# torognes/vsearch

Hardware: NVIDIA H100
Metric: usearch_global_gcups (higher is better)
Workload: dtype int16

## Files before the change

vsearch_b200/csrc/align_ckpt.cuh:

```cuda
#pragma once

#include "align_kernels.cuh"

namespace vsg {

#ifndef VSG_CK_CHUNK
#define VSG_CK_CHUNK 32
#endif
constexpr int CK_CHUNK = VSG_CK_CHUNK;
static_assert(CK_CHUNK == 16 || CK_CHUNK == 32, "chunk");

__host__ __device__ inline size_t ck_row_index(int s, int l) { return (static_cast<size_t>(s >> 2) * 32 + l) * 4 + (s & 3); }
__host__ __device__ inline size_t ck_row_elems(int dmax) { return static_cast<size_t>((dmax + 31 + 3) >> 2) * 128; }
__host__ __device__ inline size_t ck_col_index(int k, int l, int r, int R) { return (static_cast<size_t>(k - 1) * R + r) * 32 + l; }
__host__ __device__ inline size_t ck_col_elems(int dmax, int R) { return static_cast<size_t>((dmax + 31 + CK_CHUNK - 1) / CK_CHUNK) * R * 32; }

enum { CK_PROF = 0, CK_LUT = 1, CK_GEN = 2 };
__host__ __device__ constexpr size_t ck_dyn_smem(int R, int mode)
{
  return mode == CK_PROF ? static_cast<size_t>(FAST_WARPS) * 16 * ((R + 3) / 4) * 32 * 16 : 0;
}

template <int R, int MODE>
__global__ void __launch_bounds__(FAST_WARPS * 32)
nw_ckpt_kernel(const __grid_constant__ ScoreParams sp, DevSeqs qs, DevSeqs ts,
               const FastTask * __restrict__ tasks, int ntasks,
               uint2 * __restrict__ rowck, uint2 * __restrict__ colck, int32_t * __restrict__ stats)
{
  constexpr bool PROF = (MODE == CK_PROF);
  constexpr bool GENERAL = (MODE == CK_GEN);
  static_assert(!PROF || R <= 8, "the per-lane profile is for R <= 8");
  constexpr int RQ = (R + 3) / 4;
  constexpr int LUT_WORDS = GENERAL ? 4096 : (PROF ? 32 : 64 * 32);
  extern __shared__ uint4 prof_mem[];
  __shared__ uint32_t lut[LUT_WORDS];
  __shared__ uint32_t ringX[FAST_WARPS][2 * RING];
  __shared__ uint2 ringA[FAST_WARPS][2 * RING];

  int const lane = threadIdx.x & 31;
  int const wib = threadIdx.x >> 5;

  if (!PROF) {
    for (int e = threadIdx.x; e < LUT_WORDS; e += blockDim.x) {
      if (GENERAL) {
        int const q = e >> 8, dlo = e & 15, dhi = (e >> 4) & 15;
        lut[e] = pk2(-sp.S[dlo][q], -sp.S[dhi][q]);
      } else {
        int const ent = e >> 5;
        int const q = 1 << (ent >> 4), dlo = 1 << (ent & 3), dhi = 1 << ((ent >> 2) & 3);
        lut[e] = pk2(-sp.S[dlo][q], -sp.S[dhi][q]);
      }
    }
    __syncthreads();
  }

  int const w = blockIdx.x * FAST_WARPS + wib;
  if (w >= ntasks) { return; }
  FastTask const tk = tasks[w];

  int const Q = qs.len[tk.q];
  uint8_t const * __restrict__ qsym = qs.sym + qs.off[tk.q];
  int const Dlo = ts.len[tk.tlo], Dhi = ts.len[tk.thi];
  uint8_t const * __restrict__ dlo_p = ts.sym + ts.off[tk.tlo];
  uint8_t const * __restrict__ dhi_p = ts.sym + ts.off[tk.thi];
  int const dmax = tk.dmax;
  int const nsteps = dmax + 31;

  int const QRqi = sp.go[Q_I] + sp.ge[Q_I], Rqi = sp.ge[Q_I];
  int const QRqr = sp.go[Q_R] + sp.ge[Q_R], Rqr = sp.ge[Q_R];
  int const QRti = sp.go[T_I] + sp.ge[T_I], Rti = sp.ge[T_I];
  int const QRtr = sp.go[T_R] + sp.ge[T_R], Rtr = sp.ge[T_R];
  int const gotl = sp.go[T_L], getl = sp.ge[T_L];
  int const goql = sp.go[Q_L], geql = sp.ge[Q_L];
// ... 117 lines not shown
      __syncwarp();
      if (lane < CK_CHUNK && cc + CK_CHUNK < dmax) { fetch(cc + CK_CHUNK); }
    }
    uint32_t const slot0 = static_cast<uint32_t>(s0 - lane) & (RING - 1);
    constexpr unsigned CH = CK_CHUNK;
    bool const steady = (s0 >= 32) && (s0 + CK_CHUNK - 1 < dmax) &&
                        (static_cast<unsigned>(cap_lo - s0) >= CH) && (static_cast<unsigned>(cap_hi - s0) >= CH) &&
                        (static_cast<unsigned>(Dlo - 1 - (s0 - 31)) >= 31u + CH) && (static_cast<unsigned>(Dhi - 1 - (s0 - 31)) >= 31u + CH);
    if (steady) {
      bool const lo_done = (s0 - 31 > Dlo - 1), hi_done = (s0 - 31 > Dhi - 1);
      uint32_t const yneg = pk2(-(lo_done ? QRtr : QRti), -(hi_done ? QRtr : QRti));
      uint32_t const z = pk2(lo_done ? Rtr : Rti, hi_done ? Rtr : Rti);
      uint32_t const ypos = pk2(lo_done ? QRtr : QRti, hi_done ? QRtr : QRti);
      uint32_t htop = BIAS2 - pk1(goql + (s0 - lane + 1) * geql);
      uint32_t aX = rX_s + slot0 * 4u;
#pragma unroll 1
      for (int k0 = 0; k0 < CK_CHUNK; k0 += 4) {
        uint32_t ho[4], fo[4];
#pragma unroll
        for (int u = 0; u < 4; u++) {
          uint32_t hin = __shfl_up_sync(0xffffffffu, Hout, 1);
          uint32_t fin = __shfl_up_sync(0xffffffffu, Fout, 1);
          uint32_t const x = lds32(aX + (k0 + u) * 4u);
          if (lane == 0) { hin = htop; fin = htop - ypos; }
          htop -= geql2;
          column(x, yneg, z, hin, fin);
          ho[u] = Hout; fo[u] = Fout;
        }
        uint4 * const tp = reinterpret_cast<uint4 *>(myrow + ck_row_index(s0 + k0, lane));
        tp[0] = make_uint4(ho[0], fo[0], ho[1], fo[1]);
        tp[1] = make_uint4(ho[2], fo[2], ho[3], fo[3]);
      }
    } else {
      int const kend = min(CK_CHUNK, nsteps - s0);
      int c = s0 - lane;
      uint32_t aX = rX_s + slot0 * 4u, aA = rA_s + slot0 * 8u;
      for (int k = 0; k < kend; k++, c++, aX += 4u, aA += 8u) {
        uint32_t hin = __shfl_up_sync(0xffffffffu, Hout, 1);
        uint32_t fin = __shfl_up_sync(0xffffffffu, Fout, 1);
        if (c >= 0 && c < dmax) {
          uint32_t const x = lds32(aX);
          uint2 yz;
          asm volatile("ld.shared.v2.u32 {%0,%1}, [%2];" : "=r"(yz.x), "=r"(yz.y) : "r"(aA));
          if (lane == 0) {
            hin = BIAS2 - pk1(goql + (c + 1) * geql);
            fin = __vadd2(hin, yz.x);
          }
          column(x, yz.x, yz.y, hin, fin);
          myrow[ck_row_index(s0 + k, lane)] = make_uint2(Hout, Fout);
          if (capture && (c == Dlo - 1 || c == Dhi - 1)) {
            uint32_t v = 0;
#pragma unroll
            for (int r = 0; r < R; r++) { if (r == rlast) { v = Hl[r]; } }
            if (c == Dlo - 1) { score_lo = static_cast<int>(v & 0xffffu) - static_cast<int>(BIAS); }
            if (c == Dhi - 1) { score_hi = static_cast<int>(v >> 16) - static_cast<int>(BIAS); }
          }
        }
      }
    }
    if (s0 + CK_CHUNK < nsteps) {
      uint2 * const cp = mycol + ck_col_index(s0 / CK_CHUNK + 1, lane, 0, R);
#pragma unroll
      for (int r = 0; r < R; r++) { cp[static_cast<size_t>(r) * 32] = make_uint2(Hl[r], E[r]); }
    }
  }
  if (lane == llast) {
    if (tk.out_lo >= 0) { stats[static_cast<size_t>(tk.out_lo) * VSG_STAT_WORDS + VSG_STAT_SCORE] = score_lo + sp.shift * (Q + Dlo); }
    if (tk.out_hi >= 0) { stats[static_cast<size_t>(tk.out_hi) * VSG_STAT_WORDS + VSG_STAT_SCORE] = score_hi + sp.shift * (Q + Dhi); }
  }
}

}

#include "tb_ckpt.h"

namespace vsg {

static_assert(ckpt::CHUNK == CK_CHUNK && ckpt::RMAX == FAST_RMAX, "tb_ckpt.h and align_ckpt.cuh disagree");

constexpr int TB_CK_THREADS = 128;

// ... 63 lines not shown
  CigarWriter cw;
  cw.text = TEXT;
  cw.end = TEXT ? (cigar_region + pv.Q + pv.D + 1) : nullptr;
  if (TEXT) { *--cw.end = 0; }
  cw.op = 0; cw.run = 0; cw.len = 0;
  ckpt::TbOut o;
  auto emit = [&](char nop, int n) { if (TEXT) { cw.push_n(nop, n); } };
  if (general) { ckpt::traceback<RT, true>(sp, pv, bits, rows, o, emit); }
  else { ckpt::traceback<RT, false>(sp, pv, bits, rows, o, emit); }
  if (TEXT) { cw.flush(); }
  st[VSG_STAT_ALIGNED] = o.aligned; st[VSG_STAT_MATCHES] = o.matches; st[VSG_STAT_MISMATCHES] = o.mismatches;
  st[VSG_STAT_GAPS] = o.gaps; st[VSG_STAT_TRIM_LEFT] = o.trim_left; st[VSG_STAT_TRIM_RIGHT] = o.trim_right;
  st[VSG_STAT_CIGARLEN] = TEXT ? cw.len : 0;
}

constexpr int32_t TB_VERDICT_ACCEPTED = 0x5ca1ab1e;
struct TbGate {
  const int * ids;
  int nids;
  const int32_t * leader_of;
  int phase;
  int iddef;
  double threshold;
};

__device__ __forceinline__ bool tb_leader_accepted(const ckpt::TbOut & o, int Q, int D, int iddef, double threshold)
{
  int const nal = o.aligned, ma = o.matches, mi = o.mismatches, ga = o.gaps;
  int const tql = o.trim_left > 0 ? o.trim_left : 0, ttl = o.trim_left < 0 ? -o.trim_left : 0;
  int tqr = o.trim_right > 0 ? o.trim_right : 0, ttr = o.trim_right < 0 ? -o.trim_right : 0;
  if (tql >= nal) { tqr = 0; }
// ... 101 lines not shown
```

vsearch_b200/csrc/search.cu:

```cuda
#include "vsg_internal.h"
#include "hit_logic.h"

#include <algorithm>
#include <atomic>
#include <cmath>
#include <climits>
#include <cstdint>
#include <cstdlib>
#include <cstring>
#include <thread>
#include <chrono>
#include <cstdio>

namespace vsg {
int rank_enqueue(vsg_ctx * c, const vsg_index * ix, const vsg_seqset * queries, int64_t q0, int64_t nq,
                 int minwordmatches, int tophits, int mask_lower, uint32_t ** d_seqno, uint32_t ** d_count,
                 int32_t ** d_n, int32_t ** d_status);
int seqset_revcomp(vsg_ctx * c, const vsg_seqset * src, int64_t q0, int64_t nq, vsg_seqset ** out);
void rank_collect_time(vsg_ctx * c);
const vsg_seqset * index_db(const vsg_index * ix);
int index_wordlength(const vsg_index * ix);
}

using namespace vsg;
// ... 90 lines not shown
  if (opts->wordlength != index_wordlength(ix)) { Error::set("vsg_search_batch: wordlength differs from the index"); return VSG_EINVAL; }
  if (opts->iddef < 0 || opts->iddef > 4) { Error::set("vsg_search_batch: iddef must be 0..4"); return VSG_EINVAL; }

  int64_t const seqcount = db->d.n;
  int64_t maxaccepts = opts->maxaccepts, maxrejects = opts->maxrejects < 0 ? 32 : opts->maxrejects;
  if (maxaccepts < 0) { Error::set("vsg_search_batch: maxaccepts must not be negative"); return VSG_EINVAL; }
  if (maxaccepts > seqcount || maxaccepts == 0) { maxaccepts = seqcount; }
  if (maxrejects > seqcount || maxrejects == 0) { maxrejects = seqcount; }
  int64_t tophits64 = maxaccepts + maxrejects + MAXDELAYED;
  if (tophits64 > seqcount) { tophits64 = seqcount; }
  int const minwordmatches = opts->minwordmatches < 0 ? minwordmatches_defaults[opts->wordlength] : opts->minwordmatches;
  double const opt_id = opts->id;
  double const opt_weak_id = (opts->id >= 0.0 && opts->weak_id > opts->id) ? opts->id : opts->weak_id;
  int64_t total_pairs = 0, total_cells = 0, aligned_pairs = 0, aligned_cells = 0;
  bool const lazy = opts->lazy != 0;
  bool const tb_force = [] { const char * e = std::getenv("VSG_TB_GATE_FORCE"); return e != nullptr && e[0] == '1'; }();
  bool tb_gate = false;
  {
    vsg_search_opts d;
    vsg_search_opts_default(&d);
    const char * const e = std::getenv("VSG_TB_GATE");
    tb_gate = (e == nullptr || e[0] != '0') && !lazy && !c->sp.fallback &&
              opts->maxsubs == d.maxsubs && opts->maxgaps == d.maxgaps && opts->mincols == d.mincols && opts->maxdiffs == d.maxdiffs &&
              opts->leftjust == 0 && opts->rightjust == 0 && opts->query_cov == d.query_cov && opts->target_cov == d.target_cov &&
              opts->maxid == d.maxid && opts->mid == d.mid && opts->iddef >= 0 && opts->iddef <= 4 && opt_weak_id <= opt_id &&
              opts->unoise == 0;
  }
  for (int64_t q = 0; q < nq; q++) { counts[q] = 0; }
  if (seqcount == 0 || nq == 0) { if (work) { work[0] = work[1] = work[2] = work[3] = 0; } return VSG_OK; }
  if (tophits64 > 1024) { Error::set("vsg_search_batch: maxaccepts+maxrejects+8 > 1024 is not supported on the device ranker"); return VSG_EINVAL; }
  int const tophits = static_cast<int>(tophits64);
// ... 243 lines not shown
          split = 0;
          while (split < n && static_cast<int64_t>(state_of[split]) < bn) { split++; }
        }
        for (int part = 0; part < 2; part++) {
          size_t const lo = part == 0 ? 0 : split, hi = part == 0 ? split : n;
          if (hi <= lo) { continue; }
          const vsg_seqset * qset = part == 0 ? queries : rc_set;
          const int32_t * lead_part = nullptr;
          if (lead != nullptr) {
            lead_tmp.assign(lead + lo, lead + hi);
            if (lo > 0) { for (auto & v : lead_tmp) { if (v >= 0) { v -= static_cast<int32_t>(lo); } } }
            lead_part = lead_tmp.data();
          }
          int const r = align_pairs_gated(c, qset, db, static_cast<int64_t>(hi - lo), Q + lo, T + lo,
                                          o_sc + lo, o_al + lo, o_ma + lo, o_mi + lo, o_ga + lo, o_tr + 4 * lo, nullptr, 0, nullptr,
                                          lead_part, tb_force ? -1.0 : 100.0 * opt_id + 1e-7, opts->iddef);
          if (r != VSG_OK) { return r; }
        }
        return VSG_OK;
      };
      bool const from_cache = tail_mode;
      auto count_extras = [&]() -> size_t {
        size_t extras = 0;
        for (size_t k = 0; k < np; k++) {
          if (k + 1 == np || pstate[k + 1] != pstate[k]) {
            QState const & S = st[static_cast<size_t>(pstate[k])];
            extras += static_cast<size_t>(std::max(0, S.ncand - (lazy ? S.gend : S.hit_count)));
          }
        }
        return extras;
      };
// ... 386 lines not shown
```

vsearch_b200/csrc/vsg_api.cu:

```cuda
#include "align_kernels.cuh"
#include "align_ckpt.cuh"

#include <cub/cub.cuh>

#include <algorithm>
#include <atomic>
#include <cstdio>
#include <cstdlib>
#include <cstring>
#include <map>
#include <mutex>
#include <chrono>

namespace vsg {

static thread_local std::string g_last_error;
void Error::set(const std::string & m) { g_last_error = m; }

static std::atomic<int64_t> g_launches{0};
void count_launch(int n) { g_launches.fetch_add(n, std::memory_order_relaxed); }

namespace {
struct PoolKey { int device; size_t cls; bool operator<(const PoolKey & o) const { return device != o.device ? device < o.device : cls < o.cls; } };
std::mutex g_pool_mutex;
// ... 215 lines not shown
    return VSG_ECUDA;
  }
  *out = guard.release();
  return VSG_OK;
}

extern "C" void vsg_ctx_destroy(vsg_ctx * c)
{
  if (c == nullptr) { return; }
  for (vsg_ctx * ch : c->children) { vsg_ctx_destroy(ch); }
  c->children.clear();
  cudaSetDevice(c->device);
  if (c->stream != nullptr) { cudaStreamSynchronize(c->stream); }
  for (DevBuf * b : {&c->dir, &c->bnd, &c->he, &c->cigar_scratch, &c->cigar_dense, &c->stats,
                     &c->tasks_fast, &c->tasks_exact, &c->pairs, &c->cigar_len, &c->cigar_offs,
                     &c->cub_tmp, &c->rank_tmp, &c->rank_scratch, &c->pre_flags, &c->ticket}) { b->release(); }
  for (PinBuf * b : {&c->h_tasks, &c->h_stats}) { b->release(); }
  for (auto & ev : c->ev) { if (ev != nullptr) { cudaEventDestroy(ev); } }
  for (auto & ev : c->ev_pool) { cudaEventDestroy(ev); }
  if (c->stream != nullptr) { cudaStreamDestroy(c->stream); }
  delete c;
}

extern "C" int vsg_ctx_set_fallback(vsg_ctx * c, vsg_fallback_fn fn, void * user)
{
  if (c == nullptr) { return VSG_EINVAL; }
  c->fallback = fn;
  c->fallback_user = user;
  return VSG_OK;
}

// ... 161 lines not shown
    return;
  }
  switch (R) {
#define VSG_CASE(r) case r: launch_fast_one<r, false, false>(c, qs, ts, d_tasks, n); break;
    VSG_CASE(1) VSG_CASE(2) VSG_CASE(3) VSG_CASE(4) VSG_CASE(5) VSG_CASE(6) VSG_CASE(7) VSG_CASE(8)
#undef VSG_CASE
#define VSG_CASE(r) case r: if (multi) { launch_fast_one<r, false, true>(c, qs, ts, d_tasks, n); } \
                            else { launch_fast_one<r, false, false>(c, qs, ts, d_tasks, n); } break;
    VSG_CASE(9) VSG_CASE(10) VSG_CASE(11) VSG_CASE(12) VSG_CASE(13) VSG_CASE(14) VSG_CASE(15)
    default: if (multi) { launch_fast_one<16, false, true>(c, qs, ts, d_tasks, n); }
             else { launch_fast_one<16, false, false>(c, qs, ts, d_tasks, n); } break;
#undef VSG_CASE
  }
}

template <int R, int MODE>
void launch_ckpt_one(vsg_ctx * c, const DevSeqs & qs, const DevSeqs & ts, const FastTask * d_tasks, int n)
{
  int const blocks = (n + FAST_WARPS - 1) / FAST_WARPS;
  constexpr size_t dyn = ck_dyn_smem(R, MODE);
  if (dyn > 48 * 1024) {
    cudaFuncSetAttribute(nw_ckpt_kernel<R, MODE>, cudaFuncAttributeMaxDynamicSharedMemorySize, static_cast<int>(dyn));
  }
  nw_ckpt_kernel<R, MODE><<<blocks, FAST_WARPS * 32, dyn, c->stream>>>(
      c->sp2, qs, ts, d_tasks, n, static_cast<uint2 *>(c->dir.p), static_cast<uint2 *>(c->bnd.p),
      static_cast<int32_t *>(c->stats.p));
  count_launch();
}

void launch_ckpt(vsg_ctx * c, int R, bool general, const DevSeqs & qs, const DevSeqs & ts, const FastTask * d_tasks, int n)
{
  if (general) {
    switch (R) {
      case 4: launch_ckpt_one<4, CK_GEN>(c, qs, ts, d_tasks, n); break;
      case 8: launch_ckpt_one<8, CK_GEN>(c, qs, ts, d_tasks, n); break;
      default: launch_ckpt_one<16, CK_GEN>(c, qs, ts, d_tasks, n); break;
    }
    return;
  }
  static const bool force_lut = std::getenv("VSG_CK_LUT") != nullptr;
  if (force_lut && R == 8) { launch_ckpt_one<8, CK_LUT>(c, qs, ts, d_tasks, n); return; }
  switch (R) {
#define VSG_CASE(r) case r: launch_ckpt_one<r, CK_PROF>(c, qs, ts, d_tasks, n); break;
    VSG_CASE(1) VSG_CASE(2) VSG_CASE(3) VSG_CASE(4) VSG_CASE(5) VSG_CASE(6) VSG_CASE(7) VSG_CASE(8)
#undef VSG_CASE
#define VSG_CASE(r) case r: launch_ckpt_one<r, CK_LUT>(c, qs, ts, d_tasks, n); break;
    VSG_CASE(9) VSG_CASE(10) VSG_CASE(11) VSG_CASE(12) VSG_CASE(13) VSG_CASE(14) VSG_CASE(15)
    default: launch_ckpt_one<16, CK_LUT>(c, qs, ts, d_tasks, n); break;
#undef VSG_CASE
  }
}

int launch_tb_ckpt_tasks(vsg_ctx * c, int R, bool general, const DevSeqs & qs, const DevSeqs & ts, const FastTask * d_tasks, int n,
                         const TbGate & gate)
{
  int rc;
  if ((rc = c->ticket.reserve(64)) != VSG_OK) { return rc; }
  VSG_CUDA_OK(cudaMemsetAsync(c->ticket.p, 0, sizeof(int), c->stream));
  int sms = 132;
  cudaDeviceGetAttribute(&sms, cudaDevAttrMultiProcessorCount, c->device);
  int const nthr = gate.ids != nullptr ? gate.nids : 2 * n;
  if (nthr == 0) { return VSG_OK; }
  int const want = (nthr + TB_CK_THREADS - 1) / TB_CK_THREADS;
// ... 8 lines not shown
        c->sp2, qs, ts, d_tasks, n, R, general ? 1 : 0, static_cast<const uint2 *>(c->dir.p), static_cast<const uint2 *>(c->bnd.p),
        static_cast<int32_t *>(c->stats.p), static_cast<int *>(c->ticket.p), tbase, gate);
  } else {
    cudaFuncSetAttribute(traceback_ckpt_tasks_kernel<16>, cudaFuncAttributeMaxDynamicSharedMemorySize, static_cast<int>(tb_ck_smem(16)));
    int per_sm = 1;
    cudaOccupancyMaxActiveBlocksPerMultiprocessor(&per_sm, traceback_ckpt_tasks_kernel<16>, TB_CK_THREADS, tb_ck_smem(16));
    int const blocks = refill > 0 ? std::min(want, std::max(1, per_sm) * sms * refill) : want;
    traceback_ckpt_tasks_kernel<16><<<blocks, TB_CK_THREADS, tb_ck_smem(16), c->stream>>>(
        c->sp2, qs, ts, d_tasks, n, R, general ? 1 : 0, static_cast<const uint2 *>(c->dir.p), static_cast<const uint2 *>(c->bnd.p),
        static_cast<int32_t *>(c->stats.p), static_cast<int *>(c->ticket.p), tbase, gate);
  }
  count_launch();
  return VSG_OK;
}

struct ClassRun { int R; bool general, multi, ckpt; size_t first; int count; };
struct ChunkPlan {
  std::vector<ClassRun> runs;
  size_t exact_first = 0; int exact_count = 0;
  size_t pair_first = 0; int pair_count = 0;
  uint64_t dir_bytes = 0, bnd_elems = 0, he_elems = 0, cigar_bytes = 0;
  int64_t cells = 0, nfast = 0, nexact = 0;
};

struct ChunkBuilder {
  std::vector<FastTask> fast[2][3][FAST_RMAX + 1];
  std::vector<ExactTask> exact;
  uint64_t dir_bytes = 0, bnd_elems = 0, he_elems = 0, cigar_bytes = 0;
  int64_t cells = 0, nfast = 0, nexact = 0;
  int npairdesc = 0;
  bool empty() const { return nfast == 0 && nexact == 0; }
};

inline uint64_t align_up(uint64_t v, uint64_t a) { return (v + a - 1) / a * a; }

}

extern "C" int vsg_align_pairs(vsg_ctx * c, const vsg_seqset * queries, const vsg_seqset * targets,
                               int64_t npairs, const uint32_t * qidx, const uint32_t * tidx,
                               int16_t * score, uint16_t * aligned, uint16_t * matches,
                               uint16_t * mismatches, uint16_t * gaps, int32_t * trims,
// ... 27 lines not shown
  int rc;
  if ((rc = c->h_stats.reserve(sizeof(int32_t) * VSG_STAT_WORDS * static_cast<size_t>(npairs))) != VSG_OK) { return rc; }
  if ((rc = c->stats.reserve(sizeof(int32_t) * VSG_STAT_WORDS * static_cast<size_t>(npairs) + 64)) != VSG_OK) { return rc; }
  int32_t * const hs = static_cast<int32_t *>(c->h_stats.p);
  struct HostPair { int64_t slot; int32_t st[VSG_STAT_WORDS]; };
  std::vector<HostPair> host_pairs;
  std::vector<std::string> cigars;
  if (want_cigar) { cigars.resize(static_cast<size_t>(npairs)); }

  ScoreParams const & sp = c->sp;
  FastBound const fbound = fast_bound_of(sp);
  FastBound const fbound2 = fast_bound_of(c->sp2);
  const char * const ckpt_min_env = std::getenv("VSG_CKPT_MIN_PAIRS");
  int64_t const ckpt_min_pairs = ckpt_min_env != nullptr ? std::atoll(ckpt_min_env) : 2048LL;
  bool const ckpt_any_size = c->ckpt_enabled && npairs >= ckpt_min_pairs;
  std::vector<FastTask> all_fast;
  std::vector<ExactTask> all_exact;
  std::vector<PairDesc> all_pairs;
  std::vector<ChunkPlan> plans;
  ChunkBuilder cb;
  all_fast.reserve(static_cast<size_t>(npairs) / 2 + 16);
  struct Cand { int64_t slot; uint32_t t; int32_t d; bool general; };
  std::vector<Cand> group_fast;

  auto host_pair = [&](int64_t slot) -> int32_t * {
    host_pairs.emplace_back();
    host_pairs.back().slot = slot;
    std::memset(host_pairs.back().st, 0, sizeof(int32_t) * VSG_STAT_WORDS);
    return host_pairs.back().st;
  };

  auto close_chunk = [&]() {
    if (cb.empty()) { return; }
    ChunkPlan pl;
    for (int gm = 0; gm < 6; gm++) {
      int const g = gm / 3, m = gm % 3;
      for (int R = 1; R <= FAST_RMAX; R++) {
        auto & v = cb.fast[g][m][R];
        if (v.empty()) { continue; }
        auto const longer = [](const FastTask & a, const FastTask & b) { return a.dmax > b.dmax; };
        if (!std::is_sorted(v.begin(), v.end(), longer)) { std::sort(v.begin(), v.end(), longer); }
        pl.runs.push_back(ClassRun{R, g != 0, m == 1, m == 2, all_fast.size(), static_cast<int>(v.size())});
        all_fast.insert(all_fast.end(), v.begin(), v.end());
        v.clear();
      }
    }
    pl.exact_first = all_exact.size(); pl.exact_count = static_cast<int>(cb.exact.size());
    all_exact.insert(all_exact.end(), cb.exact.begin(), cb.exact.end());
    cb.exact.clear();
    pl.pair_first = all_pairs.size() - static_cast<size_t>(cb.npairdesc); pl.pair_count = cb.npairdesc;
    pl.dir_bytes = cb.dir_bytes; pl.bnd_elems = cb.bnd_elems; pl.he_elems = cb.he_elems; pl.cigar_bytes = cb.cigar_bytes;
    pl.cells = cb.cells; pl.nfast = cb.nfast; pl.nexact = cb.nexact;
    plans.push_back(std::move(pl));
    cb.dir_bytes = cb.bnd_elems = cb.he_elems = cb.cigar_bytes = 0;
    cb.cells = cb.nfast = cb.nexact = 0; cb.npairdesc = 0;
  };

// ... 74 lines not shown
        uint64_t const dirb = ck ? ck_row_elems(dmax) * sizeof(uint2) : static_cast<uint64_t>(ns) * fast_strip_bytes(dmax, R);
        uint64_t const auxe = ck ? ck_col_elems(dmax, R) : (ns > 1 ? static_cast<uint64_t>(dmax) : 0);
        if (!cb.empty() && cb.dir_bytes + dirb + (cb.bnd_elems + auxe) * sizeof(uint2) > c->dir_budget) { close_chunk(); }
        FastTask ft{};
        ft.q = q; ft.tlo = a.t; ft.thi = b.t;
        ft.out_lo = static_cast<int32_t>(a.slot);
        ft.out_hi = pair2 ? static_cast<int32_t>(b.slot) : -1;
        ft.dmax = dmax;
        ft.dir_off = ck ? cb.dir_bytes / sizeof(uint2) : cb.dir_bytes;
        ft.bnd_off = cb.bnd_elems;
        int const gbit = a.general ? 2 : 0;
        add_pairdesc(q, a.t, ck ? 2 : 0, a.slot, R, ck ? gbit : 0, dmax, ft.dir_off, ft.bnd_off);
        if (pair2) { add_pairdesc(q, b.t, ck ? 2 : 0, b.slot, R, ck ? (gbit | 1) : 1, dmax, ft.dir_off, ft.bnd_off); }
        cb.dir_bytes += align_up(dirb, 32);
        cb.bnd_elems += auxe;
        cb.fast[a.general ? 1 : 0][ck ? 2 : (ns > 1 ? 1 : 0)][R].push_back(ft);
        cb.cells += static_cast<int64_t>(Q) * a.d + (pair2 ? static_cast<int64_t>(Q) * b.d : 0);
        cb.nfast += pair2 ? 2 : 1;
        k += pair2 ? 2 : 1;
      }
    }
    i = j;
  }
  close_chunk();
  auto const t_planned = std::chrono::steady_clock::now();

  uint64_t max_dir = 0, max_bnd = 0, max_he = 0, max_cig = 0;
  for (auto const & pl : plans) {
    max_dir = std::max(max_dir, pl.dir_bytes); max_bnd = std::max(max_bnd, pl.bnd_elems);
    max_he = std::max(max_he, pl.he_elems); max_cig = std::max(max_cig, pl.cigar_bytes);
  }
// ... 47 lines not shown
    }
    if ((rc = c->gate.reserve(sizeof(int) * (ids.size() + static_cast<size_t>(npairs)) + 64)) != VSG_OK) { return rc; }
    int * const dg = static_cast<int *>(c->gate.p);
    if (!ids.empty()) { VSG_CUDA_OK(cudaMemcpyAsync(dg, ids.data(), sizeof(int) * ids.size(), cudaMemcpyHostToDevice, c->stream)); }
    VSG_CUDA_OK(cudaMemcpyAsync(dg + ids.size(), leader_of, sizeof(int32_t) * static_cast<size_t>(npairs), cudaMemcpyHostToDevice, c->stream));
    d_gate_ids = dg;
    d_leader = dg + ids.size();
    VSG_CUDA_OK(cudaMemsetAsync(c->stats.p, 0xff, sizeof(int32_t) * VSG_STAT_WORDS * static_cast<size_t>(npairs), c->stream));
  }
  while (c->ev_pool.size() < 3 * plans.size()) {
    cudaEvent_t e;
    VSG_CUDA_OK(cudaEventCreate(&e));
    c->ev_pool.push_back(e);
  }

  FastTask * const d_fast = static_cast<FastTask *>(c->tasks_fast.p);
  ExactTask * const d_exact = static_cast<ExactTask *>(c->tasks_exact.p);
  int32_t * const d_stats = static_cast<int32_t *>(c->stats.p);
  uint8_t * const d_dir = static_cast<uint8_t *>(c->dir.p);

  for (size_t ci = 0; ci < plans.size(); ci++) {
    ChunkPlan const & pl = plans[ci];
    VSG_CUDA_OK(cudaEventRecord(c->ev_pool[3 * ci], c->stream));
    for (auto const & run : pl.runs) {
      if (run.ckpt) { launch_ckpt(c, run.R, run.general, queries->d, targets->d, d_fast + run.first, run.count); }
      else { launch_fast(c, run.R, run.general, run.multi, queries->d, targets->d, d_fast + run.first, run.count); }
    }
    if (pl.exact_count > 0) {
      nw_exact_kernel<<<(pl.exact_count + 63) / 64, 64, 0, c->stream>>>(sp, queries->d, targets->d, d_exact + pl.exact_first,
                                                                        pl.exact_count, d_dir, static_cast<int16_t *>(c->he.p), d_stats);
      count_launch();
    }
    VSG_CUDA_OK(cudaEventRecord(c->ev_pool[3 * ci + 1], c->stream));
    if (!want_cigar) {
      TbGate const no_gate{nullptr, 0, nullptr, 0, 2, 0.0};
      if (gated) {
        for (size_t ri = 0; ri < pl.runs.size(); ri++) {
          auto const & run = pl.runs[ri];
          if (!run.ckpt) { continue; }
          GateRun const & g = gate_runs[ci][ri];
          TbGate const g1{d_gate_ids + g.lead_first, static_cast<int>(g.lead_count), d_leader, 1, gate_iddef, gate_threshold};
          if ((rc = launch_tb_ckpt_tasks(c, run.R, run.general, queries->d, targets->d, d_fast + run.first, run.count, g1)) != VSG_OK) { return rc; }
        }
      }
      for (size_t ri = 0; ri < pl.runs.size(); ri++) {
        auto const & run = pl.runs[ri];
        if (run.ckpt) {
          if (gated) {
            GateRun const & g = gate_runs[ci][ri];
            TbGate const g2{d_gate_ids + g.foll_first, static_cast<int>(g.foll_count), d_leader, 2, gate_iddef, gate_threshold};
            if ((rc = launch_tb_ckpt_tasks(c, run.R, run.general, queries->d, targets->d, d_fast + run.first, run.count, g2)) != VSG_OK) { return rc; }
            continue;
          }
          if ((rc = launch_tb_ckpt_tasks(c, run.R, run.general, queries->d, targets->d, d_fast + run.first, run.count, no_gate)) != VSG_OK) { return rc; }
          continue;
        }
        int const nthr = 2 * run.count;
// ... 50 lines not shown
                                                    static_cast<char *>(c->cigar_scratch.p), static_cast<char *>(c->cigar_dense.p));
      count_launch();
      std::vector<int64_t> h_offs(static_cast<size_t>(np)), h_lens(static_cast<size_t>(np));
      VSG_CUDA_OK(cudaMemcpyAsync(h_offs.data(), c->cigar_offs.p, sizeof(int64_t) * np, cudaMemcpyDeviceToHost, c->stream));
      VSG_CUDA_OK(cudaMemcpyAsync(h_lens.data(), c->cigar_len.p, sizeof(int64_t) * np, cudaMemcpyDeviceToHost, c->stream));
      VSG_CUDA_OK(cudaStreamSynchronize(c->stream));
      int64_t const total = np > 0 ? h_offs[static_cast<size_t>(np) - 1] + h_lens[static_cast<size_t>(np) - 1] : 0;
      std::vector<char> dense(static_cast<size_t>(total) + 1);
      if (total > 0) {
        VSG_CUDA_OK(cudaMemcpyAsync(dense.data(), c->cigar_dense.p, static_cast<size_t>(total), cudaMemcpyDeviceToHost, c->stream));
        VSG_CUDA_OK(cudaStreamSynchronize(c->stream));
      }
      for (int p = 0; p < np; p++) { cigars[static_cast<size_t>(hpairs[p].out)] = std::string(dense.data() + h_offs[static_cast<size_t>(p)]); }
    }
  }
  if (!plans.empty()) {
    VSG_CUDA_OK(cudaMemcpyAsync(hs, d_stats, sizeof(int32_t) * VSG_STAT_WORDS * static_cast<size_t>(npairs), cudaMemcpyDeviceToHost, c->stream));
  }
  VSG_CUDA_OK(cudaStreamSynchronize(c->stream));
  VSG_CUDA_OK(cudaGetLastError());
  for (size_t ci = 0; ci < plans.size(); ci++) {
    float ms = 0.f;
    if (cudaEventElapsedTime(&ms, c->ev_pool[3 * ci], c->ev_pool[3 * ci + 1]) == cudaSuccess) { c->prof_fwd_ms += ms; }
    if (cudaEventElapsedTime(&ms, c->ev_pool[3 * ci + 1], c->ev_pool[3 * ci + 2]) == cudaSuccess) { c->prof_tb_ms += ms; }
    c->prof_cells += plans[ci].cells; c->prof_fast += plans[ci].nfast; c->prof_exact += plans[ci].nexact;
    c->prof_fwd_launches += static_cast<int64_t>(plans[ci].runs.size()) + (plans[ci].exact_count > 0 ? 1 : 0);
  }
  for (auto const & hp : host_pairs) { std::memcpy(hs + static_cast<size_t>(hp.slot) * VSG_STAT_WORDS, hp.st, sizeof(int32_t) * VSG_STAT_WORDS); }

  int64_t cpos = 0;
// ... 15 lines not shown
    if (want_cigar) {
      std::string const & cg = cigars[static_cast<size_t>(k)];
      if (cpos + static_cast<int64_t>(cg.size()) + 1 > cigar_cap) { Error::set("vsg_align_pairs: cigar buffer too small"); return VSG_ECAP; }
      cigar_off[k] = cpos;
      std::memcpy(cigar_buf + cpos, cg.c_str(), cg.size() + 1);
      cpos += static_cast<int64_t>(cg.size()) + 1;
    }
  }
  if (want_cigar) { cigar_off[npairs] = cpos; }
  if (trace) {
    auto const t_end = std::chrono::steady_clock::now();
    std::fprintf(stderr, "[vsg trace] align_pairs %lld pairs, %zu chunk(s): plan %.1f ms, total %.1f ms\n",
                 static_cast<long long>(npairs), plans.size(),
                 std::chrono::duration<double, std::milli>(t_planned - t_begin).count(),
                 std::chrono::duration<double, std::milli>(t_end - t_begin).count());
  }
  return VSG_OK;
}

namespace vsg {
__global__ void int_peak_kernel(uint32_t * out, uint32_t seed, uint32_t one, int iters)
{
  uint32_t a[8];
#pragma unroll
  for (int k = 0; k < 8; k++) { a[k] = seed * (threadIdx.x + 1) + k * 0x00030005u; }
  for (int it = 0; it < iters; it++) {
    uint32_t n[8];
#pragma unroll
    for (int k = 0; k < 8; k++) {
      if (k & 1) { asm volatile("mad.lo.u32 %0, %1, %2, %3;" : "=r"(n[k]) : "r"(a[k]), "r"(one), "r"(a[(k + 2) & 7])); }
// ... 56 lines not shown
```

vsearch_b200/csrc/vsg_internal.h:

```cpp
#pragma once

#include <cuda_runtime.h>
#include <stdint.h>
#include <memory>
#include <string>
#include <vector>

#include "../../include/vsg.h"

namespace vsg {

enum { Q_L = 0, T_L = 1, Q_I = 2, T_I = 3, Q_R = 4, T_R = 5 };

struct ScoreParams {
  int16_t S[16][16];
  int16_t go[6];
  int16_t ge[6];
  int16_t match, mismatch;
  int16_t score_min;
  int16_t n_mismatch;
  int32_t fallback;
  int32_t shift;
};

// ... 77 lines not shown
  std::vector<uint8_t> h_nonacgt;
  vsg::DevBuf b_sym, b_off, b_len;
  int device = 0;
  int64_t total = 0;
};

struct vsg_ctx {
  int device = 0;
  cudaStream_t stream = nullptr;
  vsg_scoring scoring{};
  vsg::ScoreParams sp{};
  vsg::ScoreParams sp2{};
  bool ckpt_enabled = true;
  bool fast_disabled = false;
  vsg::DevBuf dir, bnd, he, cigar_scratch, cigar_dense, stats, tasks_fast, tasks_exact, pairs,
      cigar_len, cigar_offs, cub_tmp, rank_tmp, rank_scratch, pre_flags, ticket, gate;
  vsg::PinBuf h_tasks, h_stats;
  size_t dir_budget = (size_t)64 << 30;
  cudaEvent_t ev[6] = {nullptr, nullptr, nullptr, nullptr, nullptr, nullptr};
  int64_t prof_cells = 0, prof_fast = 0, prof_exact = 0, prof_fwd_launches = 0, prof_tb_skipped = 0;
  float prof_fwd_ms = 0.f, prof_tb_ms = 0.f, prof_rank_ms = 0.f;
  bool rank_pending = false;
  std::vector<cudaEvent_t> ev_pool;
  vsg_fallback_fn fallback = nullptr;
  void * fallback_user = nullptr;
  std::vector<vsg_ctx *> children;
  std::shared_ptr<void> search_scratch;
};
```

Before: 1590.

## Run gated checkpoint alignments score-only and re-run stores only for rejected pairs

Adds a score-only variant of the checkpoint forward kernel that skips row and column checkpoint stores for tasks whose pairs have gate leaders. After the traceback gate runs, a rerun variant recomputes with stores only for tasks whose leader was not accepted. The aim is to cut global memory write traffic for most pairs, at the cost of a second forward pass for pairs that fail the gate and added template instantiations. An env knob and trace counter are also added.

Measured after the change: 1839 (median of 6 runs). 1.16x the previous value.

```diff
diff --git a/vsearch_b200/csrc/align_ckpt.cuh b/vsearch_b200/csrc/align_ckpt.cuh
--- a/vsearch_b200/csrc/align_ckpt.cuh
+++ b/vsearch_b200/csrc/align_ckpt.cuh
@@ -9,6 +9,11 @@
 #endif
 constexpr int CK_CHUNK = VSG_CK_CHUNK;
 static_assert(CK_CHUNK == 16 || CK_CHUNK == 32, "chunk");
+#ifndef VSG_CK_SO_STEPS
+#define VSG_CK_SO_STEPS 8
+#endif
+constexpr int CK_SO_STEPS = VSG_CK_SO_STEPS;
+static_assert(CK_CHUNK % CK_SO_STEPS == 0, "score-only trip");
 
 __host__ __device__ inline size_t ck_row_index(int s, int l) { return (static_cast<size_t>(s >> 2) * 32 + l) * 4 + (s & 3); }
 __host__ __device__ inline size_t ck_row_elems(int dmax) { return static_cast<size_t>((dmax + 31 + 3) >> 2) * 128; }
@@ -21,14 +26,20 @@
   return mode == CK_PROF ? static_cast<size_t>(FAST_WARPS) * 16 * ((R + 3) / 4) * 32 * 16 : 0;
 }
 
-template <int R, int MODE>
+enum { CK_STORE = 0, CK_SCOREONLY = 1, CK_RERUN = 2 };
+
+constexpr int32_t TB_VERDICT_ACCEPTED = 0x5ca1ab1e;
+
+template <int R, int MODE, int WRITE>
 __global__ void __launch_bounds__(FAST_WARPS * 32)
 nw_ckpt_kernel(const __grid_constant__ ScoreParams sp, DevSeqs qs, DevSeqs ts,
                const FastTask * __restrict__ tasks, int ntasks,
-               uint2 * __restrict__ rowck, uint2 * __restrict__ colck, int32_t * __restrict__ stats)
+               uint2 * __restrict__ rowck, uint2 * __restrict__ colck, int32_t * __restrict__ stats,
+               const int32_t * __restrict__ leader_of, int * __restrict__ rerun_count)
 {
   constexpr bool PROF = (MODE == CK_PROF);
   constexpr bool GENERAL = (MODE == CK_GEN);
+  constexpr bool STORE = (WRITE != CK_SCOREONLY);
   static_assert(!PROF || R <= 8, "the per-lane profile is for R <= 8");
   constexpr int RQ = (R + 3) / 4;
   constexpr int LUT_WORDS = GENERAL ? 4096 : (PROF ? 32 : 64 * 32);
@@ -57,6 +68,13 @@
   int const w = blockIdx.x * FAST_WARPS + wib;
   if (w >= ntasks) { return; }
   FastTask const tk = tasks[w];
+  if (WRITE == CK_RERUN) {
+    bool need = false;
+    if (tk.out_lo >= 0) { need |= stats[static_cast<size_t>(leader_of[tk.out_lo]) * VSG_STAT_WORDS + VSG_STAT_CIGARLEN] != TB_VERDICT_ACCEPTED; }
+    if (tk.out_hi >= 0) { need |= stats[static_cast<size_t>(leader_of[tk.out_hi]) * VSG_STAT_WORDS + VSG_STAT_CIGARLEN] != TB_VERDICT_ACCEPTED; }
+    if (!need) { return; }
+    if (rerun_count != nullptr && lane == 0) { atomicAdd(rerun_count, 1); }
+  }
 
   int const Q = qs.len[tk.q];
   uint8_t const * __restrict__ qsym = qs.sym + qs.off[tk.q];
@@ -204,22 +222,33 @@
       uint32_t const ypos = pk2(lo_done ? QRtr : QRti, hi_done ? QRtr : QRti);
       uint32_t htop = BIAS2 - pk1(goql + (s0 - lane + 1) * geql);
       uint32_t aX = rX_s + slot0 * 4u;
+      auto step = [&](uint32_t ax) {
+        uint32_t hin = __shfl_up_sync(0xffffffffu, Hout, 1);
+        uint32_t fin = __shfl_up_sync(0xffffffffu, Fout, 1);
+        uint32_t const x = lds32(ax);
+        if (lane == 0) { hin = htop; fin = htop - ypos; }
+        htop -= geql2;
+        column(x, yneg, z, hin, fin);
+      };
+      if (STORE) {
 #pragma unroll 1
-      for (int k0 = 0; k0 < CK_CHUNK; k0 += 4) {
-        uint32_t ho[4], fo[4];
-#pragma unroll
-        for (int u = 0; u < 4; u++) {
-          uint32_t hin = __shfl_up_sync(0xffffffffu, Hout, 1);
-          uint32_t fin = __shfl_up_sync(0xffffffffu, Fout, 1);
-          uint32_t const x = lds32(aX + (k0 + u) * 4u);
-          if (lane == 0) { hin = htop; fin = htop - ypos; }
-          htop -= geql2;
-          column(x, yneg, z, hin, fin);
-          ho[u] = Hout; fo[u] = Fout;
+        for (int k0 = 0; k0 < CK_CHUNK; k0 += 4) {
+          uint32_t ho[4], fo[4];
+#pragma unroll
+          for (int u = 0; u < 4; u++) {
+            step(aX + (k0 + u) * 4u);
+            ho[u] = Hout; fo[u] = Fout;
+          }
+          uint4 * const tp = reinterpret_cast<uint4 *>(myrow + ck_row_index(s0 + k0, lane));
+          tp[0] = make_uint4(ho[0], fo[0], ho[1], fo[1]);
+          tp[1] = make_uint4(ho[2], fo[2], ho[3], fo[3]);
         }
-        uint4 * const tp = reinterpret_cast<uint4 *>(myrow + ck_row_index(s0 + k0, lane));
-        tp[0] = make_uint4(ho[0], fo[0], ho[1], fo[1]);
-        tp[1] = make_uint4(ho[2], fo[2], ho[3], fo[3]);
+      } else {
+#pragma unroll 1
+        for (int k0 = 0; k0 < CK_CHUNK; k0 += CK_SO_STEPS, aX += CK_SO_STEPS * 4u) {
+#pragma unroll
+          for (int u = 0; u < CK_SO_STEPS; u++) { step(aX + u * 4u); }
+        }
       }
     } else {
       int const kend = min(CK_CHUNK, nsteps - s0);
@@ -237,7 +266,7 @@
             fin = __vadd2(hin, yz.x);
           }
           column(x, yz.x, yz.y, hin, fin);
-          myrow[ck_row_index(s0 + k, lane)] = make_uint2(Hout, Fout);
+          if (STORE) { myrow[ck_row_index(s0 + k, lane)] = make_uint2(Hout, Fout); }
           if (capture && (c == Dlo - 1 || c == Dhi - 1)) {
             uint32_t v = 0;
 #pragma unroll
@@ -248,13 +277,13 @@
         }
       }
     }
-    if (s0 + CK_CHUNK < nsteps) {
+    if (STORE && s0 + CK_CHUNK < nsteps) {
       uint2 * const cp = mycol + ck_col_index(s0 / CK_CHUNK + 1, lane, 0, R);
 #pragma unroll
       for (int r = 0; r < R; r++) { cp[static_cast<size_t>(r) * 32] = make_uint2(Hl[r], E[r]); }
     }
   }
-  if (lane == llast) {
+  if (WRITE != CK_RERUN && lane == llast) {
     if (tk.out_lo >= 0) { stats[static_cast<size_t>(tk.out_lo) * VSG_STAT_WORDS + VSG_STAT_SCORE] = score_lo + sp.shift * (Q + Dlo); }
     if (tk.out_hi >= 0) { stats[static_cast<size_t>(tk.out_hi) * VSG_STAT_WORDS + VSG_STAT_SCORE] = score_hi + sp.shift * (Q + Dhi); }
   }
@@ -348,7 +377,6 @@
   st[VSG_STAT_CIGARLEN] = TEXT ? cw.len : 0;
 }
 
-constexpr int32_t TB_VERDICT_ACCEPTED = 0x5ca1ab1e;
 struct TbGate {
   const int * ids;
   int nids;
diff --git a/vsearch_b200/csrc/search.cu b/vsearch_b200/csrc/search.cu
--- a/vsearch_b200/csrc/search.cu
+++ b/vsearch_b200/csrc/search.cu
@@ -128,7 +128,7 @@
   double const opt_weak_id = (opts->id >= 0.0 && opts->weak_id > opts->id) ? opts->id : opts->weak_id;
   int64_t total_pairs = 0, total_cells = 0, aligned_pairs = 0, aligned_cells = 0;
   bool const lazy = opts->lazy != 0;
-  bool const tb_force = [] { const char * e = std::getenv("VSG_TB_GATE_FORCE"); return e != nullptr && e[0] == '1'; }();
+  int const tb_force = [] { const char * e = std::getenv("VSG_TB_GATE_FORCE"); return e != nullptr && (e[0] == '1' || e[0] == '2') ? e[0] - '0' : 0; }();
   bool tb_gate = false;
   {
     vsg_search_opts d;
@@ -402,7 +402,7 @@
           }
           int const r = align_pairs_gated(c, qset, db, static_cast<int64_t>(hi - lo), Q + lo, T + lo,
                                           o_sc + lo, o_al + lo, o_ma + lo, o_mi + lo, o_ga + lo, o_tr + 4 * lo, nullptr, 0, nullptr,
-                                          lead_part, tb_force ? -1.0 : 100.0 * opt_id + 1e-7, opts->iddef);
+                                          lead_part, tb_force == 1 ? -1.0 : (tb_force == 2 ? 1e9 : 100.0 * opt_id + 1e-7), opts->iddef);
           if (r != VSG_OK) { return r; }
         }
         return VSG_OK;
diff --git a/vsearch_b200/csrc/vsg_api.cu b/vsearch_b200/csrc/vsg_api.cu
--- a/vsearch_b200/csrc/vsg_api.cu
+++ b/vsearch_b200/csrc/vsg_api.cu
@@ -253,7 +253,7 @@
   if (c->stream != nullptr) { cudaStreamSynchronize(c->stream); }
   for (DevBuf * b : {&c->dir, &c->bnd, &c->he, &c->cigar_scratch, &c->cigar_dense, &c->stats,
                      &c->tasks_fast, &c->tasks_exact, &c->pairs, &c->cigar_len, &c->cigar_offs,
-                     &c->cub_tmp, &c->rank_tmp, &c->rank_scratch, &c->pre_flags, &c->ticket}) { b->release(); }
+                     &c->cub_tmp, &c->rank_tmp, &c->rank_scratch, &c->pre_flags, &c->ticket, &c->rerun_count}) { b->release(); }
   for (PinBuf * b : {&c->h_tasks, &c->h_stats}) { b->release(); }
   for (auto & ev : c->ev) { if (ev != nullptr) { cudaEventDestroy(ev); } }
   for (auto & ev : c->ev_pool) { cudaEventDestroy(ev); }
@@ -445,39 +445,52 @@
   }
 }
 
-template <int R, int MODE>
-void launch_ckpt_one(vsg_ctx * c, const DevSeqs & qs, const DevSeqs & ts, const FastTask * d_tasks, int n)
+template <int R, int MODE, int WRITE>
+void launch_ckpt_one(vsg_ctx * c, const DevSeqs & qs, const DevSeqs & ts, const FastTask * d_tasks, int n,
+                     const int32_t * leader_of, int * rerun_count)
 {
   int const blocks = (n + FAST_WARPS - 1) / FAST_WARPS;
   constexpr size_t dyn = ck_dyn_smem(R, MODE);
   if (dyn > 48 * 1024) {
-    cudaFuncSetAttribute(nw_ckpt_kernel<R, MODE>, cudaFuncAttributeMaxDynamicSharedMemorySize, static_cast<int>(dyn));
-  }
-  nw_ckpt_kernel<R, MODE><<<blocks, FAST_WARPS * 32, dyn, c->stream>>>(
+    cudaFuncSetAttribute(nw_ckpt_kernel<R, MODE, WRITE>, cudaFuncAttributeMaxDynamicSharedMemorySize, static_cast<int>(dyn));
+  }
+  nw_ckpt_kernel<R, MODE, WRITE><<<blocks, FAST_WARPS * 32, dyn, c->stream>>>(
       c->sp2, qs, ts, d_tasks, n, static_cast<uint2 *>(c->dir.p), static_cast<uint2 *>(c->bnd.p),
-      static_cast<int32_t *>(c->stats.p));
+      static_cast<int32_t *>(c->stats.p), leader_of, rerun_count);
   count_launch();
 }
 
-void launch_ckpt(vsg_ctx * c, int R, bool general, const DevSeqs & qs, const DevSeqs & ts, const FastTask * d_tasks, int n)
+template <int R, int MODE>
+void launch_ckpt_write(vsg_ctx * c, int write, const DevSeqs & qs, const DevSeqs & ts, const FastTask * d_tasks, int n,
+                       const int32_t * leader_of, int * rerun_count)
+{
+  switch (write) {
+    case CK_SCOREONLY: launch_ckpt_one<R, MODE, CK_SCOREONLY>(c, qs, ts, d_tasks, n, leader_of, rerun_count); break;
+    case CK_RERUN: launch_ckpt_one<R, MODE, CK_RERUN>(c, qs, ts, d_tasks, n, leader_of, rerun_count); break;
+    default: launch_ckpt_one<R, MODE, CK_STORE>(c, qs, ts, d_tasks, n, leader_of, rerun_count); break;
+  }
+}
+
+void launch_ckpt(vsg_ctx * c, int R, bool general, int write, const DevSeqs & qs, const DevSeqs & ts, const FastTask * d_tasks,
+                 int n, const int32_t * leader_of = nullptr, int * rerun_count = nullptr)
 {
   if (general) {
     switch (R) {
-      case 4: launch_ckpt_one<4, CK_GEN>(c, qs, ts, d_tasks, n); break;
-      case 8: launch_ckpt_one<8, CK_GEN>(c, qs, ts, d_tasks, n); break;
-      default: launch_ckpt_one<16, CK_GEN>(c, qs, ts, d_tasks, n); break;
+      case 4: launch_ckpt_write<4, CK_GEN>(c, write, qs, ts, d_tasks, n, leader_of, rerun_count); break;
+      case 8: launch_ckpt_write<8, CK_GEN>(c, write, qs, ts, d_tasks, n, leader_of, rerun_count); break;
+      default: launch_ckpt_write<16, CK_GEN>(c, write, qs, ts, d_tasks, n, leader_of, rerun_count); break;
     }
     return;
   }
   static const bool force_lut = std::getenv("VSG_CK_LUT") != nullptr;
-  if (force_lut && R == 8) { launch_ckpt_one<8, CK_LUT>(c, qs, ts, d_tasks, n); return; }
+  if (force_lut && R == 8) { launch_ckpt_write<8, CK_LUT>(c, write, qs, ts, d_tasks, n, leader_of, rerun_count); return; }
   switch (R) {
-#define VSG_CASE(r) case r: launch_ckpt_one<r, CK_PROF>(c, qs, ts, d_tasks, n); break;
+#define VSG_CASE(r) case r: launch_ckpt_write<r, CK_PROF>(c, write, qs, ts, d_tasks, n, leader_of, rerun_count); break;
     VSG_CASE(1) VSG_CASE(2) VSG_CASE(3) VSG_CASE(4) VSG_CASE(5) VSG_CASE(6) VSG_CASE(7) VSG_CASE(8)
 #undef VSG_CASE
-#define VSG_CASE(r) case r: launch_ckpt_one<r, CK_LUT>(c, qs, ts, d_tasks, n); break;
+#define VSG_CASE(r) case r: launch_ckpt_write<r, CK_LUT>(c, write, qs, ts, d_tasks, n, leader_of, rerun_count); break;
     VSG_CASE(9) VSG_CASE(10) VSG_CASE(11) VSG_CASE(12) VSG_CASE(13) VSG_CASE(14) VSG_CASE(15)
-    default: launch_ckpt_one<16, CK_LUT>(c, qs, ts, d_tasks, n); break;
+    default: launch_ckpt_write<16, CK_LUT>(c, write, qs, ts, d_tasks, n, leader_of, rerun_count); break;
 #undef VSG_CASE
   }
 }
@@ -516,7 +529,7 @@
   return VSG_OK;
 }
 
-struct ClassRun { int R; bool general, multi, ckpt; size_t first; int count; };
+struct ClassRun { int R; bool general, multi, ckpt, scoreonly; size_t first; int count; };
 struct ChunkPlan {
   std::vector<ClassRun> runs;
   size_t exact_first = 0; int exact_count = 0;
@@ -526,7 +539,7 @@
 };
 
 struct ChunkBuilder {
-  std::vector<FastTask> fast[2][3][FAST_RMAX + 1];
+  std::vector<FastTask> fast[2][4][FAST_RMAX + 1];
   std::vector<ExactTask> exact;
   uint64_t dir_bytes = 0, bnd_elems = 0, he_elems = 0, cigar_bytes = 0;
   int64_t cells = 0, nfast = 0, nexact = 0;
@@ -584,6 +597,8 @@
   const char * const ckpt_min_env = std::getenv("VSG_CKPT_MIN_PAIRS");
   int64_t const ckpt_min_pairs = ckpt_min_env != nullptr ? std::atoll(ckpt_min_env) : 2048LL;
   bool const ckpt_any_size = c->ckpt_enabled && npairs >= ckpt_min_pairs;
+  const char * const so_env = std::getenv("VSG_CK_SCOREONLY");
+  bool const scoreonly_ok = leader_of != nullptr && !want_cigar && (so_env == nullptr || so_env[0] != '0');
   std::vector<FastTask> all_fast;
   std::vector<ExactTask> all_exact;
   std::vector<PairDesc> all_pairs;
@@ -603,14 +618,14 @@
   auto close_chunk = [&]() {
     if (cb.empty()) { return; }
     ChunkPlan pl;
-    for (int gm = 0; gm < 6; gm++) {
-      int const g = gm / 3, m = gm % 3;
+    for (int gm = 0; gm < 8; gm++) {
+      int const g = gm / 4, m = gm % 4;
       for (int R = 1; R <= FAST_RMAX; R++) {
         auto & v = cb.fast[g][m][R];
         if (v.empty()) { continue; }
         auto const longer = [](const FastTask & a, const FastTask & b) { return a.dmax > b.dmax; };
         if (!std::is_sorted(v.begin(), v.end(), longer)) { std::sort(v.begin(), v.end(), longer); }
-        pl.runs.push_back(ClassRun{R, g != 0, m == 1, m == 2, all_fast.size(), static_cast<int>(v.size())});
+        pl.runs.push_back(ClassRun{R, g != 0, m == 1, m >= 2, m == 3, all_fast.size(), static_cast<int>(v.size())});
         all_fast.insert(all_fast.end(), v.begin(), v.end());
         v.clear();
       }
@@ -715,7 +730,8 @@
         if (pair2) { add_pairdesc(q, b.t, ck ? 2 : 0, b.slot, R, ck ? (gbit | 1) : 1, dmax, ft.dir_off, ft.bnd_off); }
         cb.dir_bytes += align_up(dirb, 32);
         cb.bnd_elems += auxe;
-        cb.fast[a.general ? 1 : 0][ck ? 2 : (ns > 1 ? 1 : 0)][R].push_back(ft);
+        bool const scoreonly = ck && scoreonly_ok && leader_of[a.slot] >= 0 && (!pair2 || leader_of[b.slot] >= 0);
+        cb.fast[a.general ? 1 : 0][scoreonly ? 3 : (ck ? 2 : (ns > 1 ? 1 : 0))][R].push_back(ft);
         cb.cells += static_cast<int64_t>(Q) * a.d + (pair2 ? static_cast<int64_t>(Q) * b.d : 0);
         cb.nfast += pair2 ? 2 : 1;
         k += pair2 ? 2 : 1;
@@ -793,6 +809,18 @@
     c->ev_pool.push_back(e);
   }
 
+  int64_t n_stored = 0, n_scoreonly = 0;
+  int * d_rerun = nullptr;
+  if (trace) {
+    for (auto const & pl : plans) {
+      for (auto const & run : pl.runs) { if (run.ckpt) { (run.scoreonly ? n_scoreonly : n_stored) += run.count; } }
+    }
+    if (n_scoreonly > 0) {
+      if ((rc = c->rerun_count.reserve(64)) != VSG_OK) { return rc; }
+      d_rerun = static_cast<int *>(c->rerun_count.p);
+      VSG_CUDA_OK(cudaMemsetAsync(d_rerun, 0, sizeof(int), c->stream));
+    }
+  }
   FastTask * const d_fast = static_cast<FastTask *>(c->tasks_fast.p);
   ExactTask * const d_exact = static_cast<ExactTask *>(c->tasks_exact.p);
   int32_t * const d_stats = static_cast<int32_t *>(c->stats.p);
@@ -802,7 +830,7 @@
     ChunkPlan const & pl = plans[ci];
     VSG_CUDA_OK(cudaEventRecord(c->ev_pool[3 * ci], c->stream));
     for (auto const & run : pl.runs) {
-      if (run.ckpt) { launch_ckpt(c, run.R, run.general, queries->d, targets->d, d_fast + run.first, run.count); }
+      if (run.ckpt) { launch_ckpt(c, run.R, run.general, run.scoreonly ? CK_SCOREONLY : CK_STORE, queries->d, targets->d, d_fast + run.first, run.count); }
       else { launch_fast(c, run.R, run.general, run.multi, queries->d, targets->d, d_fast + run.first, run.count); }
     }
     if (pl.exact_count > 0) {
@@ -820,6 +848,11 @@
           GateRun const & g = gate_runs[ci][ri];
           TbGate const g1{d_gate_ids + g.lead_first, static_cast<int>(g.lead_count), d_leader, 1, gate_iddef, gate_threshold};
           if ((rc = launch_tb_ckpt_tasks(c, run.R, run.general, queries->d, targets->d, d_fast + run.first, run.count, g1)) != VSG_OK) { return rc; }
+        }
+        for (auto const & run : pl.runs) {
+          if (run.scoreonly) {
+            launch_ckpt(c, run.R, run.general, CK_RERUN, queries->d, targets->d, d_fast + run.first, run.count, d_leader, d_rerun);
+          }
         }
       }
       for (size_t ri = 0; ri < pl.runs.size(); ri++) {
@@ -900,6 +933,8 @@
       for (int p = 0; p < np; p++) { cigars[static_cast<size_t>(hpairs[p].out)] = std::string(dense.data() + h_offs[static_cast<size_t>(p)]); }
     }
   }
+  int h_rerun = 0;
+  if (d_rerun != nullptr) { VSG_CUDA_OK(cudaMemcpyAsync(&h_rerun, d_rerun, sizeof(int), cudaMemcpyDeviceToHost, c->stream)); }
   if (!plans.empty()) {
     VSG_CUDA_OK(cudaMemcpyAsync(hs, d_stats, sizeof(int32_t) * VSG_STAT_WORDS * static_cast<size_t>(npairs), cudaMemcpyDeviceToHost, c->stream));
   }
@@ -945,6 +980,10 @@
                  static_cast<long long>(npairs), plans.size(),
                  std::chrono::duration<double, std::milli>(t_planned - t_begin).count(),
                  std::chrono::duration<double, std::milli>(t_end - t_begin).count());
+    if (n_stored + n_scoreonly > 0) {
+      std::fprintf(stderr, "[vsg trace] align_pairs checkpoint tasks: %lld stored, %lld score-only, %d of them re-run with stores\n",
+                   static_cast<long long>(n_stored), static_cast<long long>(n_scoreonly), h_rerun);
+    }
   }
   return VSG_OK;
 }
diff --git a/vsearch_b200/csrc/vsg_internal.h b/vsearch_b200/csrc/vsg_internal.h
--- a/vsearch_b200/csrc/vsg_internal.h
+++ b/vsearch_b200/csrc/vsg_internal.h
@@ -115,7 +115,7 @@
   bool ckpt_enabled = true;
   bool fast_disabled = false;
   vsg::DevBuf dir, bnd, he, cigar_scratch, cigar_dense, stats, tasks_fast, tasks_exact, pairs,
-      cigar_len, cigar_offs, cub_tmp, rank_tmp, rank_scratch, pre_flags, ticket, gate;
+      cigar_len, cigar_offs, cub_tmp, rank_tmp, rank_scratch, pre_flags, ticket, gate, rerun_count;
   vsg::PinBuf h_tasks, h_stats;
   size_t dir_budget = (size_t)64 << 30;
   cudaEvent_t ev[6] = {nullptr, nullptr, nullptr, nullptr, nullptr, nullptr};
```
